# jyakaranda/A-LeGO-LOAM

Measured on AMD Instinct MI355X. Metric: scans/sec (16x1800 LiDAR) full IP->LO->LM loop, higher is better.
Workload: dtype f32/f64

## Files before the change

a-lego-loam_amd/csrc/alego_api.hip:

```cpp
#include <hip/hip_runtime.h>

#include <cmath>
#include <cstdio>
#include <cstdlib>
#include <algorithm>
#include <cstring>
#include <mutex>
#include <set>
#include <string>
#include <vector>

#include "../../include/alego_mi355x.h"
#include "dev_common.h"
#include "dev_mem.h"
#include "front_end.h"
#include "lm_ctx.h"
#include "lm_host.h"
#include "merge_math.h"
#include "thin_math.h"
#include "loop_ctx.h"
#include "pgraph.h"
#include "prof.h"
#include "reloc.h"
#include "stream_plan.h"
// ... 188 lines not shown
  d.cap_sharp = params->n_sharp * params->n_sectors;
  d.cap_lsharp = params->n_less_sharp * params->n_sectors;
  d.cap_flat = params->n_flat * params->n_sectors;
  d.st_stride = d.cap_sharp + d.cap_lsharp + d.cap_flat + d.H;
  d.sin_ax = std::sin(params->seg_alpha_x); d.cos_ax = std::cos(params->seg_alpha_x);
  d.sin_ay = std::sin(params->seg_alpha_y); d.cos_ay = std::cos(params->seg_alpha_y);
  {
    const double lo = params->sensor_mount_ang - params->ground_angle_thres, hi = params->sensor_mount_ang + params->ground_angle_thres;
    const bool ok = lo > -89.0 && hi < 89.0 && lo < hi;
    d.tan_g_lo = ok ? std::tan(lo * M_PI / 180.0) : std::nan("");
    d.tan_g_hi = ok ? std::tan(hi * M_PI / 180.0) : std::nan("");
  }
  d.h_magic = (unsigned)((1ull << 32) / (unsigned long long)d.H) + 1u;
  d.inv_res_x = 1.0 / params->ang_res_x; d.inv_res_y = 1.0 / params->ang_res_y;
  d.tan_theta = (params->seg_theta > 0.0 && params->seg_theta < 1.5) ? std::tan(params->seg_theta) : std::nan("");
  d.opt_ip_fused = env_int("ALEGO_IP_FUSED", 1) != 0;
  d.opt_ip_half = env_int("ALEGO_IP_HALF", 1) != 0;
  d.opt_cc_fused = env_int("ALEGO_CC_FUSED", 1) != 0;
  d.opt_cc_tile = env_int("ALEGO_CC_TILE", 1) != 0;
  d.opt_ip_band = env_int("ALEGO_IP_BAND", 1) != 0;
  d.opt_fe_pick1 = env_int("ALEGO_FE_PICK1", 0) != 0;
  d.opt_fe_fused = env_int("ALEGO_FE_FUSED", 1) != 0;
  d.opt_fe_cand = env_int("ALEGO_FE_CAND", 0);
  d.opt_lo_box_lds = env_int("ALEGO_LO_BOX_LDS", 1 << 20);
  d.opt_lo_grid = env_int("ALEGO_LO_GRID", 1) != 0;
  d.opt_fo_spin = env_int("ALEGO_FE_SPIN", 0);
  d.opt_fo_pad8 = env_int("ALEGO_FE_PAD8", 0) != 0;
  d.opt_map_merge = env_int("ALEGO_MAP_MERGE", 1) != 0;
  d.opt_solve_full_eval = env_int("ALEGO_SOLVE_FULL_EVAL", 0) != 0;
  d.fcap[F_SHARP] = d.cap_sharp * d.NS; d.fcap[F_LSHARP] = d.cap_lsharp * d.NS; d.fcap[F_FLAT] = d.cap_flat * d.NS; d.fcap[F_LFLAT] = d.N;
// ... 714 lines not shown

int alego_debug_check_guards(char* report, int cap) {
  std::string r;
  const int bad = guard_check(&r);
  if (report && cap > 0) { std::strncpy(report, r.c_str(), (size_t)cap - 1); report[cap - 1] = 0; }
  return bad;
}

int alego_debug_set_option(alego_handle* h, const char* name, int value) {
  if (!h || !name) return ALEGO_ERR_ARG;
  const std::string s(name);
  DevCtx& d = h->d;
  if (s == "ALEGO_CC_FUSED") d.opt_cc_fused = value != 0;
  else if (s == "ALEGO_IP_FUSED") d.opt_ip_fused = value != 0;
  else if (s == "ALEGO_IP_HALF") d.opt_ip_half = value != 0;
  else if (s == "ALEGO_CC_TILE") d.opt_cc_tile = value != 0;
  else if (s == "ALEGO_IP_BAND") {
    HIP_TRY(h, hipDeviceSynchronize());
    HIP_TRY(h, hipMemset(d.cc_size, 0, (size_t)d.n_slots * d.N * sizeof(int)));
    HIP_TRY(h, hipMemset(d.cc_rows, 0, (size_t)d.n_slots * d.N * sizeof(unsigned long long)));
    d.opt_ip_band = value != 0;
  }
  else if (s == "ALEGO_FE_PICK1") d.opt_fe_pick1 = value != 0;
  else if (s == "ALEGO_FE_FUSED") d.opt_fe_fused = value != 0;
  else if (s == "ALEGO_FE_CAND") d.opt_fe_cand = value;
  else if (s == "ALEGO_LO_BOX_LDS") d.opt_lo_box_lds = value;
  else if (s == "ALEGO_LO_GRID") d.opt_lo_grid = value != 0;
  else if (s == "ALEGO_FE_SPIN") d.opt_fo_spin = value;
  else if (s == "ALEGO_SOLVE_FULL_EVAL") d.opt_solve_full_eval = value != 0;
  else if (s == "ALEGO_FE_PAD8") d.opt_fo_pad8 = value != 0;
// ... 674 lines not shown
```

a-lego-loam_amd/csrc/dev_common.h:

```cpp
#ifndef ALEGO_DEV_COMMON_H_
#define ALEGO_DEV_COMMON_H_

#include <hip/hip_runtime.h>
#include <stdint.h>

#include "../../include/alego_params.h"
#include "wave.h"

#define IPB_NM 9
#define IP_OWNER_TAG 0x40000000

struct DevCtx {
  alego_params P;
  int n_slots, ring_len;
  int slot0, n_launch;
  int N, H, NS;
  int Pcap;
  int cap_sharp, cap_lsharp, cap_flat;
  double sin_ax, cos_ax, sin_ay, cos_ay;
  double inv_res_x, inv_res_y;
  const double2* ip_rowtab;
  const double2* ip_coltab;
  const double* ip_colfrac;
  int ip_cmin, ip_ncb, ip_fast;
  unsigned h_magic;
  double tan_g_lo, tan_g_hi;
  double tan_theta;
  int opt_ip_fused;
  int opt_ip_half;
  int opt_cc_fused;
  int opt_cc_tile;
  int opt_fe_pick1;
  int opt_fe_fused;
  int opt_fe_cand;
  int opt_lo_box_lds;
  int opt_map_merge;
  int opt_solve_full_eval;
  float4* in_pts;
  int* in_n;
  const float4* bag_pts;
  const int* bag_n;
  const int2* bag_src;
  int n_bags, bag_len, replay_bag;
  int fs_cur, fs_last;
  int* owner;
  float* range_img;
  uint8_t* flag_img;
  int* parent;
  int* cc_size;
  unsigned long long* cc_rows;
  unsigned long long* ipb_col;
// ... 170 lines not shown
```

a-lego-loam_amd/csrc/ip_common.h:

```cpp
#ifndef ALEGO_IP_COMMON_H_
#define ALEGO_IP_COMMON_H_
#include "dev_common.h"

DEV_INLINE int ip_point_cell(const DevCtx& d, const float4 p, bool* valid_out) {
  const alego_params& P = d.P;
  bool valid;
  int cell = -1;
    const bool finite = isfinite(p.x) && isfinite(p.y) && isfinite(p.z);
    valid = finite || P.input_is_dense != 0;
    if (valid && P.near_filter) {
      const float th = (float)P.near_thres;
      if (p.x * p.x + p.y * p.y + p.z * p.z < th * th) valid = false;
    }
    if (valid && finite) {
      int row = -1, col = -1;
      bool slow = true;
      {
        const float h2 = p.x * p.x + p.y * p.y, hf = __builtin_amdgcn_sqrtf(h2);
        bool okr = (d.ip_fast & 1) && hf > 1e-3f && hf < 1e6f && fabsf(p.z) < 1e6f;
        const float t = p.z * __builtin_amdgcn_rcpf(hf), t2 = t * t;
        okr = okr && fabsf(t) < 0.6f;
        const float a = t * (0.99997726f + t2 * (-0.33262347f + t2 * (0.19354346f + t2 * (-0.11643287f + t2 * (0.05265332f + t2 * -0.01172120f)))));
        const float r0 = (a * 57.29577951f + (float)P.ang_bottom) * (float)d.inv_res_y + 0.5f;
        const float kf = floorf(r0);
// ... 142 lines not shown
  }
  const bool live = valid && finite;
  const bool dec = live && c.fast && ok;
  const int row = rfl >= 0 ? rfl : (rfl == -1 ? 0 : -1);
  col = col >= c.H ? col - c.H : col;
  const bool in = row >= 0 && row < c.NS && col >= 0 && col < c.H;
  *valid_out = valid;
  *cell_out = (dec && in) ? col + row * c.H : -1;
  return !live || dec;
}
DEV_INLINE void ip_quick_margins(const DevCtx& d, float* mr, float* mc) {
  *mr = fmaxf(0.005f, 8e-6f * 57.29577951f * (float)d.inv_res_y + 1e-5f);
  *mc = fmaxf(0.02f, 8e-6f * 57.29577951f * (float)d.inv_res_x + 8e-7f * (float)d.H);
}

__device__ __attribute__((noinline)) inline bool ip_is_ground_ref(double dx, double dy, double dz, double mount, double thres) {
  const double angle = (atan2(dz, hypot(dx, dy)) * 180.0) / M_PI;
  return fabs(angle - mount) < thres;
}
__device__ __attribute__((noinline)) inline bool edge_angle_ref(double y, double x, double theta) { return atan2(y, x) > theta; }
DEV_INLINE int ip_ground_margins(double tan_lo, double tan_hi, float fx, float fy, float fz) {
  const double dx = (double)fx, dy = (double)fy, dz = (double)fz;
  const double h2 = dx * dx + dy * dy, z2 = dz * dz;
  const double l2 = (tan_lo * tan_lo) * h2, u2 = (tan_hi * tan_hi) * h2;
  const double sz = copysign(z2, dz);
  const double m1 = sz - copysign(l2, tan_lo), m2 = copysign(u2, tan_hi) - sz;
  const double t1 = 1e-9 * (z2 + l2), t2 = 1e-9 * (z2 + u2);
  const bool yes = m1 > t1 && m2 > t2, no = m1 < -t1 || m2 < -t2;
  return yes ? 1 : (no ? 0 : -1);
}
DEV_INLINE bool ip_is_ground(const DevCtx& d, float fx, float fy, float fz) {
  const int g = ip_ground_margins(d.tan_g_lo, d.tan_g_hi, fx, fy, fz);
  if (g >= 0) return g != 0;
  return ip_is_ground_ref((double)fx, (double)fy, (double)fz, d.P.sensor_mount_ang, d.P.ground_angle_thres);
}

DEV_INLINE int edge_angle_margin(double y, double x, double tan_theta) {
  const double xt = x * tan_theta, m = y - xt;
  return fabs(m) > 1e-9 * (y + fabs(xt)) ? (m > 0.0 ? 1 : 0) : -1;
}
DEV_INLINE bool edge_angle_gt(double y, double x, double theta, double tan_theta) {
  const double xt = x * tan_theta, m = y - xt;
  if (fabs(m) > 1e-9 * (y + fabs(xt))) return m > 0.0;
  return edge_angle_ref(y, x, theta);
}


DEV_INLINE int ccl16_find(uint16_t* par, int v) {
  int curr = par[v];
  if (curr != v) {
    int prev = v, next;
    while (curr > (next = par[curr])) { par[prev] = (uint16_t)next; prev = curr; curr = next; }
  }
  return curr;
}
DEV_INLINE int ccl16_cas(uint16_t* par, int idx, int expect, int val) {
  unsigned* w = reinterpret_cast<unsigned*>(par) + (idx >> 1);
  const int sh = (idx & 1) * 16;
  unsigned old = __hip_atomic_load(w, __ATOMIC_RELAXED, __HIP_MEMORY_SCOPE_WORKGROUP);
// ... 24 lines not shown
```

a-lego-loam_amd/csrc/kernels_ipb.hip:

```cpp
#include <cstdlib>
#include "dev_common.h"
#include "front_end.h"
#include "ip_common.h"
#include "prof.h"

#define IPB_TW 256
#define IPB_NWV (IPB_TW / 64)
#ifndef IPB_MT
#define IPB_MT 512
#endif
#define IPB_LINK_CAP 1024
#define IPB_ET 256
#ifndef IPB_EP
#define IPB_EP 4
#endif

typedef unsigned long long u64;
#ifdef ALEGO_TIMING
__device__ long long ipb_times[48];
extern "C" void alego_ipb_times(long long* out) { (void)hipMemcpyFromSymbol(out, HIP_SYMBOL(ipb_times), sizeof(long long) * 48); }
#define IPB_TICK(k) do { if (threadIdx.x == 0 && blockIdx.x == 0 && blockIdx.y == 0) ipb_times[k] = wall_clock64(); } while (0)
#else
#define IPB_TICK(k)
#endif
DEV_INLINE u64 ipb_low(int r) { return (2ull << r) - 1ull; }
DEV_INLINE int ipb_head(u64 rs, int r) { return 63 - __clzll((long long)(rs & ipb_low(r))); }
DEV_INLINE int ipb_ld(const int* p) { return __hip_atomic_load(p, __ATOMIC_RELAXED, __HIP_MEMORY_SCOPE_AGENT); }
DEV_INLINE u64 ipb_ld64(const u64* p) { return __hip_atomic_load(p, __ATOMIC_RELAXED, __HIP_MEMORY_SCOPE_AGENT); }
DEV_INLINE void ipb_st(int* p, int v) { __hip_atomic_store(p, v, __ATOMIC_RELAXED, __HIP_MEMORY_SCOPE_AGENT); }

DEV_INLINE int ipb_find(int* parent, int v) {
  int curr = ipb_ld(parent + v);
  if (curr != v) {
    int prev = v, next;
    while (curr > (next = ipb_ld(parent + curr))) { ipb_st(parent + prev, next); prev = curr; curr = next; }
  }
  return curr;
}
// ... 3 lines not shown
  return curr;
}
DEV_INLINE int ipb_union(int* parent, int a, int b) {
  int ra = ipb_find(parent, a), rb = ipb_find(parent, b);
  bool repeat;
  int linked = -1;
  do {
    repeat = false;
    if (ra != rb) {
      int ret;
      if (ra < rb) { if ((ret = atomicCAS(parent + rb, rb, ra)) != rb) { rb = ret; repeat = true; } else linked = rb; }
      else { if ((ret = atomicCAS(parent + ra, ra, rb)) != ra) { ra = ret; repeat = true; } else linked = ra; }
    }
  } while (repeat);
  return linked;
}
DEV_INLINE bool ipb_feasible(const alego_params& P, int sz, u64 rows) {
  return sz >= P.seg_big_num || (sz >= P.seg_valid_point_num && (int)__popcll(rows) >= P.seg_valid_line_num);
}

__global__ void __launch_bounds__(IPB_TW) ipb_band(DevCtx d, int ring_pos, int keep) {
  const int slot = blockIdx.y + d.slot0, tid = threadIdx.x, lane = tid & 63, wave = tid >> 6;
  const int H = d.H, NS = d.NS, c0 = blockIdx.x * IPB_TW;
  const int TW = min(IPB_TW, H - c0);
  const bool have = tid < TW;
  const int col = have ? c0 + tid : c0;
  const size_t base = (size_t)slot * d.N;
  const alego_params& P = d.P;
  const float4* pts = scan_pts(d, slot, ring_pos);
  __shared__ uint16_t par[IPB_TW * 64];
// ... 6 lines not shown
    sc[SC_PVALID_OUT] = sc[SC_PVALID];
    sc[SC_FIRST] = 0x7fffffff; sc[SC_LAST] = -1; sc[SC_PVALID] = 0;
    if (last >= 0) {
      const float4 p0 = pts[first], p1 = pts[last];
      float so = -d_atan2f(p0.y, p0.x);
      float eo = (float)((double)(-d_atan2f(p1.y, p1.x)) + 2 * M_PI);
      if ((double)(eo - so) > 3 * M_PI) eo = (float)((double)eo - 2 * M_PI);
      else if ((double)(eo - so) < M_PI) eo = (float)((double)eo + 2 * M_PI);
      ori[0] = so; ori[1] = eo; ori[2] = eo - so;
    }
  }
  IPB_TICK(0);
  int* owner = d.owner + base;
  float rng[64];
  u64 filled = 0, ground = 0;
  {
    float lx = 0, ly = 0, lz = 0;
    bool lower_ok = false;
    int obn[8];
#pragma unroll
    for (int u = 0; u < 8; ++u) obn[u] = (have && u < NS) ? owner[u * H + col] : -1;
#pragma unroll
    for (int row0 = 0; row0 < 64; row0 += 8) {
      if (row0 < NS) {
        int ob[8];
        float4 pb[8];
#pragma unroll
        for (int u = 0; u < 8; ++u) ob[u] = obn[u];
        if (row0 + 8 < 64 && row0 + 8 < NS) {
#pragma unroll
          for (int u = 0; u < 8; ++u) obn[u] = (have && row0 + 8 + u < NS) ? owner[(row0 + 8 + u) * H + col] : -1;
// ... 1 lines not shown
#pragma unroll
        for (int u = 0; u < 8; ++u) {
          ob[u] = (ob[u] >= 0 && (ob[u] & IP_OWNER_TAG)) ? (ob[u] & ~IP_OWNER_TAG) : -1;
          if (have && tid != 0 && row0 + u < NS) owner[(row0 + u) * H + col] = ob[u];
        }
#pragma unroll
        for (int u = 0; u < 8; ++u) pb[u] = pts[max(ob[u], 0)];
#pragma unroll
        for (int u = 0; u < 8; ++u) {
          const int row = row0 + u;
          const bool ok = ob[u] >= 0;
          const float x = pb[u].x, y = pb[u].y, z = pb[u].z;
          const float r = ok ? sqrtf(x * x + y * y + z * z) : -1.0f;
          rng[row] = r;
          if (ok) filled |= 1ull << row;
          if (row >= 1 && row - 1 < P.ground_scan_id && ok && lower_ok) {
            if (ip_is_ground(d, x - lx, y - ly, z - lz)) ground |= 3ull << (row - 1);
          }
          lx = x; ly = y; lz = z; lower_ok = ok;
          if ((keep & 1) && have && row < NS) d.range_img[base + row * H + col] = r;
        }
      } else {
#pragma unroll
        for (int u = 0; u < 8; ++u) rng[row0 + u] = -1.0f;
      }
    }
  }
  IPB_TICK(1);
  const u64 act = filled & ~ground;
  if (have) s_a[tid] = act;
  if (lane == 0) {
#pragma unroll
    for (int row = 0; row < 64; ++row) s_first[wave][row] = rng[row];
  }
  if (wave == 0) {
    const int hc = (c0 + TW == H) ? 0 : c0 + TW;
    int o = lane < NS ? owner[lane * H + hc] : -1;
    o = (o >= 0 && (o & IP_OWNER_TAG)) ? (o & ~IP_OWNER_TAG) : -1;
    const float4 p = pts[max(o, 0)];
    const bool ok = o >= 0;
    const float px = __shfl_up(p.x, 1, 64), py = __shfl_up(p.y, 1, 64), pz = __shfl_up(p.z, 1, 64);
    const int okl = __shfl_up(ok ? 1 : 0, 1, 64);
    bool gp = false;
    if (lane >= 1 && lane - 1 < P.ground_scan_id && ok && okl) gp = ip_is_ground(d, p.x - px, p.y - py, p.z - pz);
    const u64 gb = __ballot(gp), fb = __ballot(ok);
    s_first[IPB_NWV][lane] = ok ? sqrtf(p.x * p.x + p.y * p.y + p.z * p.z) : -1.0f;
    if (lane == 0) s_a[TW] = fb & ~(gb | (gb >> 1));
  }
  __syncthreads();
  IPB_TICK(2);
  u64 ex = 0, ey = 0;
  {
    const u64 act_r = s_a[min(tid + 1, TW)];
    const bool edge_lane = lane == 63 || tid == TW - 1;
    const float* sf = s_first[(tid >= TW - 1) ? IPB_NWV : wave + 1];
#pragma unroll
    for (int row = 0; row < 64; ++row) {
      const float nbd = __int_as_float(__builtin_amdgcn_update_dpp(0, __float_as_int(rng[row]), 0x130, 0xF, 0xF, false));
      const float nbl = sf[row];
      const float nb = edge_lane ? nbl : nbd;
      if ((act >> row) & 1ull) {
        const double r0 = (double)rng[row];
        if ((act_r >> row) & 1ull) {
          const double r1 = (double)nb;
          const double d1 = fmax(r0, r1), d2 = fmin(r0, r1);
          if (edge_angle_gt(d2 * d.sin_ax, d1 - d2 * d.cos_ax, P.seg_theta, d.tan_theta)) ex |= 1ull << row;
        }
        if (row + 1 < 64 && ((act >> (row + 1)) & 1ull)) {
          const double r1 = (double)rng[row + 1 < 64 ? row + 1 : 63];
          const double d1 = fmax(r0, r1), d2 = fmin(r0, r1);
          if (edge_angle_gt(d2 * d.sin_ay, d1 - d2 * d.cos_ay, P.seg_theta, d.tan_theta)) ey |= 1ull << row;
        }
      }
    }
  }
  if (H <= 1) ex = 0;
  IPB_TICK(3);
  const u64 rs = act & ~(ey << 1);
  s_y[tid] = ey; s_rs[tid] = rs;
  for (u64 m = rs; m; m &= m - 1) { const int r = __ffsll((long long)m) - 1; par[r * IPB_TW + tid] = (uint16_t)(r * IPB_TW + tid); }
  __syncthreads();
  IPB_TICK(4);
  if (tid + 1 < TW) {
    const u64 rs_n = s_rs[tid + 1], ey_n = s_y[tid + 1];
    for (u64 m = ex & ~((ex << 1) & (ey << 1) & (ey_n << 1)); m; m &= m - 1) {
      const int r = __ffsll((long long)m) - 1;
// ... 225 lines not shown
```

a-lego-loam_amd/csrc/kernels_ipf.hip:

```cpp
#include <type_traits>
#include <algorithm>
#include <cstdlib>
#include "dev_common.h"
#include "front_end.h"
#include "ip_common.h"
#include "prof.h"

#define IPF2_T 1024
#ifndef IPF_QUICK
#define IPF_QUICK 1
#endif
#define IPF2_NW (IPF2_T / 64)
#define IPF2_ROWS 16

struct IpfShared {
  float first_r[IPF2_NW][IPF2_ROWS];
  unsigned first_act[IPF2_NW];
  int red[3][IPF2_NW];
  int cnt[3][IPF2_ROWS * IPF2_NW];
  int wtot[3][4];
  int tot[3];
  int nlist;
};

#ifdef ALEGO_TIMING
__device__ long long ipf_times[16];
#define IPF_TICK(k) do { if (threadIdx.x == 0 && blockIdx.x == 0) ipf_times[k] = wall_clock64(); } while (0)
extern "C" void alego_ipf_times(long long* out) { (void)hipMemcpyFromSymbol(out, HIP_SYMBOL(ipf_times), sizeof(long long) * 16); }
#else
#define IPF_TICK(k)
#endif

DEV_INLINE int ipf_run_start(unsigned rs, int row) { return 31 - __clz((int)(rs & ((2u << row) - 1u))); }
DEV_INLINE int ipf_run_end(unsigned down, int s) { return s + __ffs((int)~(down >> s)) - 1; }

bool ipf_eligible(const DevCtx& d) { return d.NS <= IPF2_ROWS && (d.H & 1) == 0 && d.H >= 64 && d.H <= 2 * IPF2_T && d.N <= 32768; }
size_t ipf_lds_bytes(const DevCtx& d) { return (size_t)4 * d.N + (size_t)8 * d.H; }

__global__ void __launch_bounds__(IPF2_T) ip_fused(DevCtx d, int ring_pos, int keep) {
  const int slot = blockIdx.x + d.slot0;
  const int tid = threadIdx.x, lane = tid & 63, wave = tid >> 6;
  const int N = d.N, H = d.H, NS = d.NS;
  const size_t base = (size_t)slot * N;
  const alego_params& P = d.P;
  extern __shared__ __attribute__((aligned(16))) unsigned char ipf_smem[];
// ... 422 lines not shown
#else
static size_t iph_pad() { return 0; }
#endif

DEV_INLINE void iph_max16(unsigned* w32, int cell, unsigned val) {
  unsigned* w = w32 + (cell >> 1);
  const int sh = (cell & 1) * 16;
  unsigned old = __hip_atomic_load(w, __ATOMIC_RELAXED, __HIP_MEMORY_SCOPE_WORKGROUP);
  while (((old >> sh) & 0xFFFFu) < val) {
    const unsigned nw = (old & ~(0xFFFFu << sh)) | (val << sh);
    const unsigned got = atomicCAS(w, old, nw);
    if (got == old) break;
    old = got;
  }
}
struct IphCol { unsigned a, b, x, y; };
DEV_INLINE IphCol iph_load(const unsigned long long* fcol, int c) { const unsigned long long v = fcol[c]; IphCol m; m.a = (unsigned)v & 0xFFFFu; m.b = (unsigned)(v >> 16) & 0xFFFFu; m.x = (unsigned)(v >> 32) & 0xFFFFu; m.y = (unsigned)(v >> 48); return m; }
DEV_INLINE void iph_store(unsigned long long* fcol, int c, const IphCol& m) { fcol[c] = (unsigned long long)m.a | ((unsigned long long)m.b << 16) | ((unsigned long long)m.x << 32) | ((unsigned long long)m.y << 48); }

#ifdef IPH_STOP_AFTER
#define IPH_STOP(k) do { if ((k) == IPH_STOP_AFTER) return; } while (0)
#else
#define IPH_STOP(k)
#endif
#ifndef IPH_MINW
#define IPH_MINW 4
#endif
template <int T, int NP>
__global__ void __launch_bounds__(T, IPH_MINW) ip_fused_t(DevCtx d, int ring_pos, int keep) {
  constexpr int NW = T / 64;
  const int slot = blockIdx.x + d.slot0;
  const int tid = threadIdx.x, lane = tid & 63, wave = tid >> 6;
  const int N = d.N, H = d.H, NS = d.NS;
  const size_t base = (size_t)slot * N;
  const alego_params& P = d.P;
  extern __shared__ __attribute__((aligned(16))) unsigned char ipf_smem[];
  unsigned* own16w = reinterpret_cast<unsigned*>(ipf_smem);
  uint16_t* par = reinterpret_cast<uint16_t*>(ipf_smem);
  unsigned long long* fcol = reinterpret_cast<unsigned long long*>(ipf_smem + (size_t)2 * N);
  unsigned* own_g = d.ipf_own + (size_t)slot * (N / 2);
  __shared__ IphShared<NW, NP> S;
  const int hpairs = H / 2;
  IPF_TICK(0);
  for (int v = tid; v < N / 2; v += T) own16w[v] = 0u;
  if (tid == 0) S.nlist = 0;
  __syncthreads();
  const int n = scan_count(d, slot, ring_pos);
  const float4* pts = scan_pts(d, slot, ring_pos);
  { IPH_PHASE_CTX;
  {
// ... 101 lines not shown
      else if ((double)(eo - so) < M_PI) eo = (float)((double)eo + 2 * M_PI);
      ori[0] = so; ori[1] = eo; ori[2] = eo - so;
    }
  }

  }
  IPH_STOP(1);
  IPF_TICK(1);
  { IPH_PHASE_CTX;
#pragma unroll 1
  for (int p = 0; p < NP; ++p) {
    const int pi = tid + p * T, c0 = 2 * pi, c1 = c0 + 1;
    const bool colv = pi < hpairs;
    float rng0[IPF2_ROWS], rng1[IPF2_ROWS];
    unsigned filled0 = 0, filled1 = 0, ground0 = 0, ground1 = 0;
    {
      float lx0 = 0, ly0 = 0, lz0 = 0, lx1 = 0, ly1 = 0, lz1 = 0;
      bool lok0 = false, lok1 = false;
#pragma unroll
      for (int row0 = 0; row0 < IPF2_ROWS; row0 += IPH_GB) {
        unsigned ob[IPH_GB];
        float4 pa[IPH_GB], pb[IPH_GB];
#pragma unroll
        for (int u = 0; u < IPH_GB; ++u) ob[u] = (colv && row0 + u < NS) ? own16w[((row0 + u) * H + c0) >> 1] : 0u;
#pragma unroll
        for (int u = 0; u < IPH_GB; ++u) { pa[u] = pts[max((int)(ob[u] & 0xFFFFu) - 1, 0)]; pb[u] = pts[max((int)(ob[u] >> 16) - 1, 0)]; }
#pragma unroll
        for (int u = 0; u < IPH_GB; ++u) {
          const int row = row0 + u;
          if (colv && row < NS) own_g[(row * H + c0) >> 1] = ob[u];
          {
            const bool ok = (ob[u] & 0xFFFFu) != 0u;
            const float x = pa[u].x, y = pa[u].y, z = pa[u].z;
            rng0[row] = ok ? sqrtf(x * x + y * y + z * z) : -1.0f;
            if (ok) filled0 |= 1u << row;
            if (row >= 1 && row - 1 < P.ground_scan_id && ok && lok0 && ip_is_ground(d, x - lx0, y - ly0, z - lz0)) ground0 |= 3u << (row - 1);
            lx0 = x; ly0 = y; lz0 = z; lok0 = ok;
          }
          {
            const bool ok = (ob[u] >> 16) != 0u;
            const float x = pb[u].x, y = pb[u].y, z = pb[u].z;
            rng1[row] = ok ? sqrtf(x * x + y * y + z * z) : -1.0f;
            if (ok) filled1 |= 1u << row;
            if (row >= 1 && row - 1 < P.ground_scan_id && ok && lok1 && ip_is_ground(d, x - lx1, y - ly1, z - lz1)) ground1 |= 3u << (row - 1);
            lx1 = x; ly1 = y; lz1 = z; lok1 = ok;
          }
        }
      }
    }
    const unsigned act0 = filled0 & ~ground0, act1 = filled1 & ~ground1;
    __syncthreads();
    if (lane == 0) {
#pragma unroll
      for (int r = 0; r < IPF2_ROWS; ++r) S.u.b.first_r[wave][r] = rng0[r];
      S.u.b.first_act[wave] = act0;
    }
    if (p == 0 && tid == 0) {
#pragma unroll
      for (int r = 0; r < IPF2_ROWS; ++r) S.col0_r[r] = rng0[r];
      S.col0_act = act0;
    }
    {
      const int pil = (T - 1) + p * T;
      if (p + 1 < NP && pil < hpairs - 1 && wave == NW - 1 && lane < IPF2_ROWS) {
        const int row = lane, cx = 2 * pil + 2;
        const unsigned ow = row < NS ? (own16w[(row * H + cx) >> 1] & 0xFFFFu) : 0u;
        const float4 q = pts[max((int)ow - 1, 0)];
        const bool ok = ow != 0u;
        const float lx = __shfl_up(q.x, 1, 64), ly = __shfl_up(q.y, 1, 64), lz = __shfl_up(q.z, 1, 64);
        const bool lok = __shfl_up(ok ? 1 : 0, 1, 64) != 0;
        const bool g = row >= 1 && row - 1 < P.ground_scan_id && ok && lok && ip_is_ground(d, q.x - lx, q.y - ly, q.z - lz);
        const unsigned gm = (unsigned)__ballot(g) & 0xFFFFu, fm = (unsigned)__ballot(ok) & 0xFFFFu;
        S.np.np_r[row] = ok ? sqrtf(q.x * q.x + q.y * q.y + q.z * q.z) : -1.0f;
        if (lane == 0) S.np.np_act = fm & ~(gm | (gm >> 1));
      }
    }
    __syncthreads();
    float nbr[IPF2_ROWS];
    unsigned nb_act = (unsigned)__shfl_down((int)act0, 1, 64);
#pragma unroll
    for (int r = 0; r < IPF2_ROWS; ++r) nbr[r] = __shfl_down(rng0[r], 1, 64);
    const bool wrap = pi == hpairs - 1;
    const bool nextpass = !wrap && tid == T - 1 && p + 1 < NP;
    if ((lane == 63 && !nextpass) || wrap) {
      const int sw = min(wave + 1, NW - 1);
#pragma unroll
      for (int r = 0; r < IPF2_ROWS; ++r) nbr[r] = wrap ? S.col0_r[r] : S.u.b.first_r[sw][r];
      nb_act = wrap ? S.col0_act : S.u.b.first_act[sw];
    }
    if (nextpass) {
#pragma unroll
      for (int r = 0; r < IPF2_ROWS; ++r) nbr[r] = S.np.np_r[r];
      nb_act = S.np.np_act;
    }
    unsigned redge0 = 0, redge1 = 0, down0 = 0, down1 = 0;
    if (colv) {
      double k_sax = d.sin_ax, k_cax = d.cos_ax, k_say = d.sin_ay, k_cay = d.cos_ay, k_tan = d.tan_theta, k_theta = P.seg_theta;
      asm volatile("" : "+s"(k_sax), "+s"(k_cax), "+s"(k_say), "+s"(k_cay), "+s"(k_tan), "+s"(k_theta));
#pragma unroll
      for (int row = 0; row < IPF2_ROWS; ++row) {
        if (row < NS) {
          if ((act0 >> row) & 1u) {
            const double r0 = (double)rng0[row];
            if ((act1 >> row) & 1u) {
              const double r1 = (double)rng1[row], d1 = fmax(r0, r1), d2 = fmin(r0, r1);
              if (edge_angle_gt(d2 * k_sax, d1 - d2 * k_cax, k_theta, k_tan)) redge0 |= 1u << row;
            }
            if (row + 1 < NS && ((act0 >> (row + 1)) & 1u)) {
              const double r1 = (double)rng0[row + 1 < IPF2_ROWS ? row + 1 : row], d1 = fmax(r0, r1), d2 = fmin(r0, r1);
              if (edge_angle_gt(d2 * k_say, d1 - d2 * k_cay, k_theta, k_tan)) down0 |= 1u << row;
            }
          }
          if ((act1 >> row) & 1u) {
            const double r0 = (double)rng1[row];
            if ((nb_act >> row) & 1u) {
              const double r1 = (double)nbr[row], d1 = fmax(r0, r1), d2 = fmin(r0, r1);
              if (edge_angle_gt(d2 * k_sax, d1 - d2 * k_cax, k_theta, k_tan)) redge1 |= 1u << row;
            }
            if (row + 1 < NS && ((act1 >> (row + 1)) & 1u)) {
              const double r1 = (double)rng1[row + 1 < IPF2_ROWS ? row + 1 : row], d1 = fmax(r0, r1), d2 = fmin(r0, r1);
              if (edge_angle_gt(d2 * k_say, d1 - d2 * k_cay, k_theta, k_tan)) down1 |= 1u << row;
            }
          }
        }
      }
      fcol[c0] = (unsigned long long)ground0 | ((unsigned long long)act0 << 16) | ((unsigned long long)redge0 << 32) | ((unsigned long long)down0 << 48);
      fcol[c1] = (unsigned long long)ground1 | ((unsigned long long)act1 << 16) | ((unsigned long long)redge1 << 32) | ((unsigned long long)down1 << 48);
      if (keep & 1) {
        float* rimg = d.range_img + base;
        uint8_t* fimg = d.flag_img + base;
#pragma unroll
        for (int row = 0; row < IPF2_ROWS; ++row) {
          if (row < NS) {
            rimg[row * H + c0] = rng0[row]; rimg[row * H + c1] = rng1[row];
            fimg[row * H + c0] = (uint8_t)(((ground0 >> row) & 1u) | (((act0 >> row) & 1u) << 1) | (((redge0 >> row) & 1u) << 2) | (((down0 >> row) & 1u) << 3));
            fimg[row * H + c1] = (uint8_t)(((ground1 >> row) & 1u) | (((act1 >> row) & 1u) << 1) | (((redge1 >> row) & 1u) << 2) | (((down1 >> row) & 1u) << 3));
          }
        }
      }
    }
// ... 305 lines not shown
```

Measured before the change: 480,300.

## Screen ground and edge-angle tests in fp32 with exact fp64 fallback

Replaces the per-cell fp64 ground-angle and edge-angle predicates in the image-projection kernels with fp32 screening tests built from host-precomputed constants and error bands. Cells the screen cannot decide confidently are collected in bitmasks and re-evaluated with the original fp64/atan2 path, reloading their points from the owner map. The aim is to cut fp64 arithmetic and divergent branching in the hot unrolled row loops, at the cost of a second, gather-based slow pass for ambiguous cells and extra register pressure.

```diff
diff --git a/a-lego-loam_amd/csrc/alego_api.hip b/a-lego-loam_amd/csrc/alego_api.hip
--- a/a-lego-loam_amd/csrc/alego_api.hip
+++ b/a-lego-loam_amd/csrc/alego_api.hip
@@ -226,6 +226,8 @@
   d.h_magic = (unsigned)((1ull << 32) / (unsigned long long)d.H) + 1u;
   d.inv_res_x = 1.0 / params->ang_res_x; d.inv_res_y = 1.0 / params->ang_res_y;
   d.tan_theta = (params->seg_theta > 0.0 && params->seg_theta < 1.5) ? std::tan(params->seg_theta) : std::nan("");
+  d.opt_ip_screen = env_int("ALEGO_IP_SCREEN", 1) != 0;
+  d.ip_scr = ip_screen_consts(d.sin_ax, d.cos_ax, d.sin_ay, d.cos_ay, d.tan_theta, d.tan_g_lo, d.tan_g_hi, d.opt_ip_screen);
   d.opt_ip_fused = env_int("ALEGO_IP_FUSED", 1) != 0;
   d.opt_ip_half = env_int("ALEGO_IP_HALF", 1) != 0;
   d.opt_cc_fused = env_int("ALEGO_CC_FUSED", 1) != 0;
@@ -970,6 +972,7 @@
   if (s == "ALEGO_CC_FUSED") d.opt_cc_fused = value != 0;
   else if (s == "ALEGO_IP_FUSED") d.opt_ip_fused = value != 0;
   else if (s == "ALEGO_IP_HALF") d.opt_ip_half = value != 0;
+  else if (s == "ALEGO_IP_SCREEN") { d.opt_ip_screen = value != 0; d.ip_scr = ip_screen_consts(d.sin_ax, d.cos_ax, d.sin_ay, d.cos_ay, d.tan_theta, d.tan_g_lo, d.tan_g_hi, d.opt_ip_screen); }
   else if (s == "ALEGO_CC_TILE") d.opt_cc_tile = value != 0;
   else if (s == "ALEGO_IP_BAND") {
     HIP_TRY(h, hipDeviceSynchronize());
diff --git a/a-lego-loam_amd/csrc/dev_common.h b/a-lego-loam_amd/csrc/dev_common.h
--- a/a-lego-loam_amd/csrc/dev_common.h
+++ b/a-lego-loam_amd/csrc/dev_common.h
@@ -6,6 +6,7 @@
 
 #include "../../include/alego_params.h"
 #include "wave.h"
+#include "ip_pred.h"
 
 #define IPB_NM 9
 #define IP_OWNER_TAG 0x40000000
@@ -26,6 +27,7 @@
   unsigned h_magic;
   double tan_g_lo, tan_g_hi;
   double tan_theta;
+  IpScreenConsts ip_scr;
   int opt_ip_fused;
   int opt_ip_half;
   int opt_cc_fused;
@@ -35,6 +37,7 @@
   int opt_fe_cand;
   int opt_lo_box_lds;
   int opt_map_merge;
+  int opt_ip_screen;
   int opt_solve_full_eval;
   float4* in_pts;
   int* in_n;
diff --git a/a-lego-loam_amd/csrc/ip_common.h b/a-lego-loam_amd/csrc/ip_common.h
--- a/a-lego-loam_amd/csrc/ip_common.h
+++ b/a-lego-loam_amd/csrc/ip_common.h
@@ -180,35 +180,8 @@
   *mc = fmaxf(0.02f, 8e-6f * 57.29577951f * (float)d.inv_res_x + 8e-7f * (float)d.H);
 }
 
-__device__ __attribute__((noinline)) inline bool ip_is_ground_ref(double dx, double dy, double dz, double mount, double thres) {
-  const double angle = (atan2(dz, hypot(dx, dy)) * 180.0) / M_PI;
-  return fabs(angle - mount) < thres;
-}
-__device__ __attribute__((noinline)) inline bool edge_angle_ref(double y, double x, double theta) { return atan2(y, x) > theta; }
-DEV_INLINE int ip_ground_margins(double tan_lo, double tan_hi, float fx, float fy, float fz) {
-  const double dx = (double)fx, dy = (double)fy, dz = (double)fz;
-  const double h2 = dx * dx + dy * dy, z2 = dz * dz;
-  const double l2 = (tan_lo * tan_lo) * h2, u2 = (tan_hi * tan_hi) * h2;
-  const double sz = copysign(z2, dz);
-  const double m1 = sz - copysign(l2, tan_lo), m2 = copysign(u2, tan_hi) - sz;
-  const double t1 = 1e-9 * (z2 + l2), t2 = 1e-9 * (z2 + u2);
-  const bool yes = m1 > t1 && m2 > t2, no = m1 < -t1 || m2 < -t2;
-  return yes ? 1 : (no ? 0 : -1);
-}
 DEV_INLINE bool ip_is_ground(const DevCtx& d, float fx, float fy, float fz) {
-  const int g = ip_ground_margins(d.tan_g_lo, d.tan_g_hi, fx, fy, fz);
-  if (g >= 0) return g != 0;
-  return ip_is_ground_ref((double)fx, (double)fy, (double)fz, d.P.sensor_mount_ang, d.P.ground_angle_thres);
-}
-
-DEV_INLINE int edge_angle_margin(double y, double x, double tan_theta) {
-  const double xt = x * tan_theta, m = y - xt;
-  return fabs(m) > 1e-9 * (y + fabs(xt)) ? (m > 0.0 ? 1 : 0) : -1;
-}
-DEV_INLINE bool edge_angle_gt(double y, double x, double theta, double tan_theta) {
-  const double xt = x * tan_theta, m = y - xt;
-  if (fabs(m) > 1e-9 * (y + fabs(xt))) return m > 0.0;
-  return edge_angle_ref(y, x, theta);
+  return ip_ground_decide(d.tan_g_lo, d.tan_g_hi, d.P.sensor_mount_ang, d.P.ground_angle_thres, fx, fy, fz);
 }
 
 
diff --git a/a-lego-loam_amd/csrc/ip_pred.h b/a-lego-loam_amd/csrc/ip_pred.h
--- /dev/null
+++ b/a-lego-loam_amd/csrc/ip_pred.h
@@ -0,0 +1,106 @@
+#ifndef ALEGO_IP_PRED_H_
+#define ALEGO_IP_PRED_H_
+
+#ifdef __HIPCC__
+#define IP_PRED_FN __device__ __forceinline__
+#define IP_PRED_REF __device__ __attribute__((noinline)) inline
+#define IP_PRED_HOST __host__ inline
+#else
+#include <math.h>
+#define IP_PRED_FN inline
+#define IP_PRED_REF inline
+#define IP_PRED_HOST inline
+#endif
+
+IP_PRED_REF bool ip_is_ground_ref(double dx, double dy, double dz, double mount, double thres) {
+  const double angle = (atan2(dz, hypot(dx, dy)) * 180.0) / M_PI;
+  return fabs(angle - mount) < thres;
+}
+IP_PRED_REF bool edge_angle_ref(double y, double x, double theta) { return atan2(y, x) > theta; }
+IP_PRED_FN int ip_ground_margins(double tan_lo, double tan_hi, float fx, float fy, float fz) {
+  const double dx = (double)fx, dy = (double)fy, dz = (double)fz;
+  const double h2 = dx * dx + dy * dy, z2 = dz * dz;
+  const double l2 = (tan_lo * tan_lo) * h2, u2 = (tan_hi * tan_hi) * h2;
+  const double sz = copysign(z2, dz);
+  const double m1 = sz - copysign(l2, tan_lo), m2 = copysign(u2, tan_hi) - sz;
+  const double t1 = 1e-9 * (z2 + l2), t2 = 1e-9 * (z2 + u2);
+  const bool yes = m1 > t1 && m2 > t2, no = m1 < -t1 || m2 < -t2;
+  return yes ? 1 : (no ? 0 : -1);
+}
+IP_PRED_FN bool ip_ground_decide(double tan_lo, double tan_hi, double mount, double thres, float fx, float fy, float fz) {
+  const int g = ip_ground_margins(tan_lo, tan_hi, fx, fy, fz);
+  if (g >= 0) return g != 0;
+  return ip_is_ground_ref((double)fx, (double)fy, (double)fz, mount, thres);
+}
+
+IP_PRED_FN int edge_angle_margin(double y, double x, double tan_theta) {
+  const double xt = x * tan_theta, m = y - xt;
+  return fabs(m) > 1e-9 * (y + fabs(xt)) ? (m > 0.0 ? 1 : 0) : -1;
+}
+IP_PRED_FN bool edge_angle_gt(double y, double x, double theta, double tan_theta) {
+  const double xt = x * tan_theta, m = y - xt;
+  if (fabs(m) > 1e-9 * (y + fabs(xt))) return m > 0.0;
+  return edge_angle_ref(y, x, theta);
+}
+
+struct IpScreenBits { bool yes, und; };
+
+#define IP_SCREEN_TINY 1e-24f
+IP_PRED_FN IpScreenBits ip_edge_screen(float d1, float d2, float kh, float kl, float band) {
+  const float p = d2 * kh, e = fmaf(d2, kh, -p), s = p - d1, E = s + fmaf(d2, kl, e);
+  const bool dec = fabsf(E) > band * d1 && d2 >= IP_SCREEN_TINY;
+  IpScreenBits r;
+  r.yes = dec && E > 0.0f;
+  r.und = !dec;
+  return r;
+}
+
+#define IP_GROUND_TOL 4e-6f
+#define IP_GROUND_FLOOR 1e-30f
+IP_PRED_FN IpScreenBits ip_ground_screen(float g_lo, float g_hi, float g_max, float fx, float fy, float fz) {
+  const float h2 = fx * fx + fy * fy, z2 = fz * fz;
+  const float sz = copysignf(z2, fz);
+  const float m1 = sz - g_lo * h2, m2 = g_hi * h2 - sz;
+  const float sum = z2 + g_max * h2, tol = IP_GROUND_TOL * sum;
+  const bool big = sum >= IP_GROUND_FLOOR;
+  const bool yes = m1 > tol && m2 > tol, no = m1 < -tol || m2 < -tol;
+  IpScreenBits r;
+  r.yes = yes && big;
+  r.und = !((yes || no) && big);
+  return r;
+}
+
+struct IpScreenConsts {
+  float kxh, kxl, kyh, kyl;
+  float eband;
+  float g_lo, g_hi, g_max;
+};
+IP_PRED_HOST double ip_edge_band(double sin_a, double cos_a, double tan_theta) {
+  if (!(tan_theta > 0.0) || !(tan_theta < 1e3) || !(sin_a > 0.0) || !(cos_a > 0.0) || !(sin_a < 1.0)) return -1.0;
+  const double K = (sin_a + cos_a * tan_theta) / tan_theta;
+  if (!(K > 1.0 / 1024.0) || !(K < 1024.0)) return -1.0;
+  const double b = 4.0 * (2.01e-9 * sin_a / tan_theta + 1e-15 * (1.0 + 1.0 / tan_theta) + 2.9e-14);
+  if (!(b < 1e-6)) return -1.0;
+  return b > 8e-9 ? b : 8e-9;
+}
+IP_PRED_HOST IpScreenConsts ip_screen_consts(double sin_ax, double cos_ax, double sin_ay, double cos_ay, double tan_theta, double tan_lo, double tan_hi, int enable) {
+  IpScreenConsts c;
+  c.kxh = c.kxl = c.kyh = c.kyl = NAN; c.eband = INFINITY;
+  c.g_lo = c.g_hi = c.g_max = NAN;
+  if (!enable) return c;
+  const double bx = ip_edge_band(sin_ax, cos_ax, tan_theta), by = ip_edge_band(sin_ay, cos_ay, tan_theta);
+  if (bx > 0.0 && by > 0.0) {
+    const double Kx = (sin_ax + cos_ax * tan_theta) / tan_theta, Ky = (sin_ay + cos_ay * tan_theta) / tan_theta;
+    c.kxh = (float)Kx; c.kxl = (float)(Kx - (double)c.kxh);
+    c.kyh = (float)Ky; c.kyl = (float)(Ky - (double)c.kyh);
+    c.eband = (float)((bx > by ? bx : by) * (1.0 + 1e-6));
+  }
+  if (tan_lo < tan_hi && fabs(tan_lo) < 1e3 && fabs(tan_hi) < 1e3) {
+    const double l2 = tan_lo * tan_lo, u2 = tan_hi * tan_hi;
+    c.g_lo = (float)copysign(l2, tan_lo); c.g_hi = (float)copysign(u2, tan_hi);
+    c.g_max = (float)((l2 > u2 ? l2 : u2) * (1.0 + 1e-6));
+  }
+  return c;
+}
+
+#endif
diff --git a/a-lego-loam_amd/csrc/kernels_ipb.hip b/a-lego-loam_amd/csrc/kernels_ipb.hip
--- a/a-lego-loam_amd/csrc/kernels_ipb.hip
+++ b/a-lego-loam_amd/csrc/kernels_ipb.hip
@@ -20,8 +20,15 @@
 __device__ long long ipb_times[48];
 extern "C" void alego_ipb_times(long long* out) { (void)hipMemcpyFromSymbol(out, HIP_SYMBOL(ipb_times), sizeof(long long) * 48); }
 #define IPB_TICK(k) do { if (threadIdx.x == 0 && blockIdx.x == 0 && blockIdx.y == 0) ipb_times[k] = wall_clock64(); } while (0)
+__device__ unsigned long long ipb_slow_cnt[4];
+#define IPB_SLOW_COUNT(k) do { if ((threadIdx.x & 63) == 0) atomicAdd(&ipb_slow_cnt[k], 1ull); } while (0)
+extern "C" void alego_ipb_slow_counts(unsigned long long* out, int reset) {
+  (void)hipMemcpyFromSymbol(out, HIP_SYMBOL(ipb_slow_cnt), sizeof(unsigned long long) * 4);
+  if (reset) { const unsigned long long z[4] = {0, 0, 0, 0}; (void)hipMemcpyToSymbol(HIP_SYMBOL(ipb_slow_cnt), z, sizeof(z)); }
+}
 #else
 #define IPB_TICK(k)
+#define IPB_SLOW_COUNT(k)
 #endif
 DEV_INLINE u64 ipb_low(int r) { return (2ull << r) - 1ull; }
 DEV_INLINE int ipb_head(u64 rs, int r) { return 63 - __clzll((long long)(rs & ipb_low(r))); }
@@ -55,6 +62,11 @@
     }
   } while (repeat);
   return linked;
+}
+DEV_INLINE float4 ipb_cell_point(const int* owner, const float4* pts, int H, int row, int col) { return pts[max(ipb_ld(owner + row * H + col), 0) & ~IP_OWNER_TAG]; }
+DEV_INLINE float ipb_cell_range(const int* owner, const float4* pts, int H, int row, int col) {
+  const float4 q = ipb_cell_point(owner, pts, H, row, col);
+  return sqrtf(q.x * q.x + q.y * q.y + q.z * q.z);
 }
 DEV_INLINE bool ipb_feasible(const alego_params& P, int sz, u64 rows) {
   return sz >= P.seg_big_num || (sz >= P.seg_valid_point_num && (int)__popcll(rows) >= P.seg_valid_line_num);
@@ -91,7 +103,11 @@
   int* owner = d.owner + base;
   float rng[64];
   u64 filled = 0, ground = 0;
+  IPB_SLOW_COUNT(0);
   {
+    float k_glo = d.ip_scr.g_lo, k_ghi = d.ip_scr.g_hi, k_gmax = d.ip_scr.g_max;
+    asm volatile("" : "+s"(k_glo), "+s"(k_ghi), "+s"(k_gmax));
+    u64 gund = 0;
     float lx = 0, ly = 0, lz = 0;
     bool lower_ok = false;
     int obn[8];
@@ -123,8 +139,11 @@
           const float r = ok ? sqrtf(x * x + y * y + z * z) : -1.0f;
           rng[row] = r;
           if (ok) filled |= 1ull << row;
-          if (row >= 1 && row - 1 < P.ground_scan_id && ok && lower_ok) {
-            if (ip_is_ground(d, x - lx, y - ly, z - lz)) ground |= 3ull << (row - 1);
+          if (row >= 1 && row - 1 < P.ground_scan_id) {
+            const IpScreenBits g = ip_ground_screen(k_glo, k_ghi, k_gmax, x - lx, y - ly, z - lz);
+            const bool en = ok && lower_ok;
+            ground |= (en && g.yes) ? 3ull << (row - 1) : 0ull;
+            gund |= (en && g.und) ? 1ull << row : 0ull;
           }
           lx = x; ly = y; lz = z; lower_ok = ok;
           if ((keep & 1) && have && row < NS) d.range_img[base + row * H + col] = r;
@@ -132,6 +151,15 @@
       } else {
 #pragma unroll
         for (int u = 0; u < 8; ++u) rng[row0 + u] = -1.0f;
+      }
+    }
+    if (__ballot(gund != 0ull)) {
+      IPB_SLOW_COUNT(1);
+#pragma unroll 1
+      for (u64 m = gund; m; m &= m - 1) {
+        const int row = __ffsll((long long)m) - 1;
+        const float4 q = ipb_cell_point(owner, pts, H, row, col), l = ipb_cell_point(owner, pts, H, row - 1, col);
+        if (ip_is_ground(d, q.x - l.x, q.y - l.y, q.z - l.z)) ground |= 3ull << (row - 1);
       }
     }
   }
@@ -150,8 +178,12 @@
     const bool ok = o >= 0;
     const float px = __shfl_up(p.x, 1, 64), py = __shfl_up(p.y, 1, 64), pz = __shfl_up(p.z, 1, 64);
     const int okl = __shfl_up(ok ? 1 : 0, 1, 64);
-    bool gp = false;
-    if (lane >= 1 && lane - 1 < P.ground_scan_id && ok && okl) gp = ip_is_ground(d, p.x - px, p.y - py, p.z - pz);
+    const IpScreenBits gs = ip_ground_screen(d.ip_scr.g_lo, d.ip_scr.g_hi, d.ip_scr.g_max, p.x - px, p.y - py, p.z - pz);
+    const bool gen = lane >= 1 && lane - 1 < P.ground_scan_id && ok && okl;
+    bool gp = gen && gs.yes;
+    if (__ballot(gen && gs.und)) {
+      if (gen && gs.und) gp = ip_is_ground(d, p.x - px, p.y - py, p.z - pz);
+    }
     const u64 gb = __ballot(gp), fb = __ballot(ok);
     s_first[IPB_NWV][lane] = ok ? sqrtf(p.x * p.x + p.y * p.y + p.z * p.z) : -1.0f;
     if (lane == 0) s_a[TW] = fb & ~(gb | (gb >> 1));
@@ -163,22 +195,42 @@
     const u64 act_r = s_a[min(tid + 1, TW)];
     const bool edge_lane = lane == 63 || tid == TW - 1;
     const float* sf = s_first[(tid >= TW - 1) ? IPB_NWV : wave + 1];
+    float k_kxh = d.ip_scr.kxh, k_kxl = d.ip_scr.kxl, k_kyh = d.ip_scr.kyh, k_kyl = d.ip_scr.kyl, k_eb = d.ip_scr.eband;
+    asm volatile("" : "+s"(k_kxh), "+s"(k_kxl), "+s"(k_kyh), "+s"(k_kyl), "+s"(k_eb));
+    u64 ux = 0, uy = 0;
 #pragma unroll
     for (int row = 0; row < 64; ++row) {
       const float nbd = __int_as_float(__builtin_amdgcn_update_dpp(0, __float_as_int(rng[row]), 0x130, 0xF, 0xF, false));
       const float nbl = sf[row];
       const float nb = edge_lane ? nbl : nbd;
-      if ((act >> row) & 1ull) {
-        const double r0 = (double)rng[row];
-        if ((act_r >> row) & 1ull) {
-          const double r1 = (double)nb;
+      const float r0 = rng[row];
+      if (__ballot((act >> row) & 1ull)) {
+        {
+          const IpScreenBits e = ip_edge_screen(fmaxf(r0, nb), fminf(r0, nb), k_kxh, k_kxl, k_eb);
+          ex |= e.yes ? 1ull << row : 0ull; ux |= e.und ? 1ull << row : 0ull;
+        }
+        if (row + 1 < 64) {
+          const float r1 = rng[row + 1 < 64 ? row + 1 : 63];
+          const IpScreenBits e = ip_edge_screen(fmaxf(r0, r1), fminf(r0, r1), k_kyh, k_kyl, k_eb);
+          ey |= e.yes ? 1ull << row : 0ull; uy |= e.und ? 1ull << row : 0ull;
+        }
+      }
+    }
+    const u64 sx = act & act_r, sy = act & (act >> 1);
+    ex &= sx; ey &= sy; ux &= sx; uy &= sy;
+    if (__ballot((ux | uy) != 0ull)) {
+      IPB_SLOW_COUNT(2);
+      const int cr = col + 1 == H ? 0 : col + 1;
+#pragma unroll 1
+      for (int k = 0; k < 2; ++k) {
+        const double sa = k ? d.sin_ay : d.sin_ax, ca = k ? d.cos_ay : d.cos_ax;
+#pragma unroll 1
+        for (u64 m = k ? uy : ux; m; m &= m - 1) {
+          const int row = __ffsll((long long)m) - 1;
+          const double r0 = (double)ipb_cell_range(owner, pts, H, row, col);
+          const double r1 = (double)(k ? ipb_cell_range(owner, pts, H, row + 1, col) : ipb_cell_range(owner, pts, H, row, cr));
           const double d1 = fmax(r0, r1), d2 = fmin(r0, r1);
-          if (edge_angle_gt(d2 * d.sin_ax, d1 - d2 * d.cos_ax, P.seg_theta, d.tan_theta)) ex |= 1ull << row;
-        }
-        if (row + 1 < 64 && ((act >> (row + 1)) & 1ull)) {
-          const double r1 = (double)rng[row + 1 < 64 ? row + 1 : 63];
-          const double d1 = fmax(r0, r1), d2 = fmin(r0, r1);
-          if (edge_angle_gt(d2 * d.sin_ay, d1 - d2 * d.cos_ay, P.seg_theta, d.tan_theta)) ey |= 1ull << row;
+          if (edge_angle_gt(d2 * sa, d1 - d2 * ca, P.seg_theta, d.tan_theta)) { if (k) ey |= 1ull << row; else ex |= 1ull << row; }
         }
       }
     }
diff --git a/a-lego-loam_amd/csrc/kernels_ipf.hip b/a-lego-loam_amd/csrc/kernels_ipf.hip
--- a/a-lego-loam_amd/csrc/kernels_ipf.hip
+++ b/a-lego-loam_amd/csrc/kernels_ipf.hip
@@ -27,8 +27,15 @@
 __device__ long long ipf_times[16];
 #define IPF_TICK(k) do { if (threadIdx.x == 0 && blockIdx.x == 0) ipf_times[k] = wall_clock64(); } while (0)
 extern "C" void alego_ipf_times(long long* out) { (void)hipMemcpyFromSymbol(out, HIP_SYMBOL(ipf_times), sizeof(long long) * 16); }
+__device__ unsigned long long iph_slow_cnt[4];
+#define IPH_SLOW_COUNT(k) do { if ((threadIdx.x & 63) == 0) atomicAdd(&iph_slow_cnt[k], 1ull); } while (0)
+extern "C" void alego_iph_slow_counts(unsigned long long* out, int reset) {
+  (void)hipMemcpyFromSymbol(out, HIP_SYMBOL(iph_slow_cnt), sizeof(unsigned long long) * 4);
+  if (reset) { const unsigned long long z[4] = {0, 0, 0, 0}; (void)hipMemcpyToSymbol(HIP_SYMBOL(iph_slow_cnt), z, sizeof(z)); }
+}
 #else
 #define IPF_TICK(k)
+#define IPH_SLOW_COUNT(k)
 #endif
 
 DEV_INLINE int ipf_run_start(unsigned rs, int row) { return 31 - __clz((int)(rs & ((2u << row) - 1u))); }
@@ -481,6 +488,14 @@
     old = got;
   }
 }
+DEV_INLINE float4 iph_cell_point(const unsigned* own16w, const float4* pts, int H, int row, int col) {
+  const unsigned ow = (own16w[(row * H + col) >> 1] >> ((col & 1) * 16)) & 0xFFFFu;
+  return pts[max((int)ow - 1, 0)];
+}
+DEV_INLINE float iph_cell_range(const unsigned* own16w, const float4* pts, int H, int row, int col) {
+  const float4 q = iph_cell_point(own16w, pts, H, row, col);
+  return sqrtf(q.x * q.x + q.y * q.y + q.z * q.z);
+}
 struct IphCol { unsigned a, b, x, y; };
 DEV_INLINE IphCol iph_load(const unsigned long long* fcol, int c) { const unsigned long long v = fcol[c]; IphCol m; m.a = (unsigned)v & 0xFFFFu; m.b = (unsigned)(v >> 16) & 0xFFFFu; m.x = (unsigned)(v >> 32) & 0xFFFFu; m.y = (unsigned)(v >> 48); return m; }
 DEV_INLINE void iph_store(unsigned long long* fcol, int c, const IphCol& m) { fcol[c] = (unsigned long long)m.a | ((unsigned long long)m.b << 16) | ((unsigned long long)m.x << 32) | ((unsigned long long)m.y << 48); }
@@ -500,7 +515,6 @@
   const int tid = threadIdx.x, lane = tid & 63, wave = tid >> 6;
   const int N = d.N, H = d.H, NS = d.NS;
   const size_t base = (size_t)slot * N;
-  const alego_params& P = d.P;
   extern __shared__ __attribute__((aligned(16))) unsigned char ipf_smem[];
   unsigned* own16w = reinterpret_cast<unsigned*>(ipf_smem);
   uint16_t* par = reinterpret_cast<uint16_t*>(ipf_smem);
@@ -632,7 +646,11 @@
     const bool colv = pi < hpairs;
     float rng0[IPF2_ROWS], rng1[IPF2_ROWS];
     unsigned filled0 = 0, filled1 = 0, ground0 = 0, ground1 = 0;
+    IPH_SLOW_COUNT(0);
     {
+      float k_glo = d.ip_scr.g_lo, k_ghi = d.ip_scr.g_hi, k_gmax = d.ip_scr.g_max;
+      asm volatile("" : "+s"(k_glo), "+s"(k_ghi), "+s"(k_gmax));
+      unsigned gund = 0;
       float lx0 = 0, ly0 = 0, lz0 = 0, lx1 = 0, ly1 = 0, lz1 = 0;
       bool lok0 = false, lok1 = false;
 #pragma unroll
@@ -652,7 +670,12 @@
             const float x = pa[u].x, y = pa[u].y, z = pa[u].z;
             rng0[row] = ok ? sqrtf(x * x + y * y + z * z) : -1.0f;
             if (ok) filled0 |= 1u << row;
-            if (row >= 1 && row - 1 < P.ground_scan_id && ok && lok0 && ip_is_ground(d, x - lx0, y - ly0, z - lz0)) ground0 |= 3u << (row - 1);
+            if (row >= 1 && row - 1 < P.ground_scan_id) {
+              const IpScreenBits g = ip_ground_screen(k_glo, k_ghi, k_gmax, x - lx0, y - ly0, z - lz0);
+              const bool en = ok && lok0;
+              ground0 |= (en && g.yes) ? 3u << (row - 1) : 0u;
+              gund |= (en && g.und) ? 1u << row : 0u;
+            }
             lx0 = x; ly0 = y; lz0 = z; lok0 = ok;
           }
           {
@@ -660,9 +683,23 @@
             const float x = pb[u].x, y = pb[u].y, z = pb[u].z;
             rng1[row] = ok ? sqrtf(x * x + y * y + z * z) : -1.0f;
             if (ok) filled1 |= 1u << row;
-            if (row >= 1 && row - 1 < P.ground_scan_id && ok && lok1 && ip_is_ground(d, x - lx1, y - ly1, z - lz1)) ground1 |= 3u << (row - 1);
+            if (row >= 1 && row - 1 < P.ground_scan_id) {
+              const IpScreenBits g = ip_ground_screen(k_glo, k_ghi, k_gmax, x - lx1, y - ly1, z - lz1);
+              const bool en = ok && lok1;
+              ground1 |= (en && g.yes) ? 3u << (row - 1) : 0u;
+              gund |= (en && g.und) ? 0x10000u << row : 0u;
+            }
             lx1 = x; ly1 = y; lz1 = z; lok1 = ok;
           }
+        }
+      }
+      if (__ballot(gund != 0u)) {
+        IPH_SLOW_COUNT(1);
+#pragma unroll 1
+        for (unsigned m = gund; m; m &= m - 1) {
+          const int b = __ffs((int)m) - 1, row = b & 15, c = c0 + (b >> 4);
+          const float4 q = iph_cell_point(own16w, pts, H, row, c), l = iph_cell_point(own16w, pts, H, row - 1, c);
+          if (ip_is_ground(d, q.x - l.x, q.y - l.y, q.z - l.z)) { if (b >> 4) ground1 |= 3u << (row - 1); else ground0 |= 3u << (row - 1); }
         }
       }
     }
@@ -687,7 +724,12 @@
         const bool ok = ow != 0u;
         const float lx = __shfl_up(q.x, 1, 64), ly = __shfl_up(q.y, 1, 64), lz = __shfl_up(q.z, 1, 64);
         const bool lok = __shfl_up(ok ? 1 : 0, 1, 64) != 0;
-        const bool g = row >= 1 && row - 1 < P.ground_scan_id && ok && lok && ip_is_ground(d, q.x - lx, q.y - ly, q.z - lz);
+        const IpScreenBits gs = ip_ground_screen(d.ip_scr.g_lo, d.ip_scr.g_hi, d.ip_scr.g_max, q.x - lx, q.y - ly, q.z - lz);
+        const bool gen = row >= 1 && row - 1 < P.ground_scan_id && ok && lok;
+        bool g = gen && gs.yes;
+        if (__ballot(gen && gs.und)) {
+          if (gen && gs.und) g = ip_is_ground(d, q.x - lx, q.y - ly, q.z - lz);
+        }
         const unsigned gm = (unsigned)__ballot(g) & 0xFFFFu, fm = (unsigned)__ballot(ok) & 0xFFFFu;
         S.np.np_r[row] = ok ? sqrtf(q.x * q.x + q.y * q.y + q.z * q.z) : -1.0f;
         if (lane == 0) S.np.np_act = fm & ~(gm | (gm >> 1));
@@ -712,36 +754,62 @@
       nb_act = S.np.np_act;
     }
     unsigned redge0 = 0, redge1 = 0, down0 = 0, down1 = 0;
+    unsigned ux0 = 0, ux1 = 0, uy0 = 0, uy1 = 0;
     if (colv) {
-      double k_sax = d.sin_ax, k_cax = d.cos_ax, k_say = d.sin_ay, k_cay = d.cos_ay, k_tan = d.tan_theta, k_theta = P.seg_theta;
-      asm volatile("" : "+s"(k_sax), "+s"(k_cax), "+s"(k_say), "+s"(k_cay), "+s"(k_tan), "+s"(k_theta));
+      float k_kxh = d.ip_scr.kxh, k_kxl = d.ip_scr.kxl, k_kyh = d.ip_scr.kyh, k_kyl = d.ip_scr.kyl, k_eb = d.ip_scr.eband;
+      asm volatile("" : "+s"(k_kxh), "+s"(k_kxl), "+s"(k_kyh), "+s"(k_kyl), "+s"(k_eb));
 #pragma unroll
       for (int row = 0; row < IPF2_ROWS; ++row) {
-        if (row < NS) {
-          if ((act0 >> row) & 1u) {
-            const double r0 = (double)rng0[row];
-            if ((act1 >> row) & 1u) {
-              const double r1 = (double)rng1[row], d1 = fmax(r0, r1), d2 = fmin(r0, r1);
-              if (edge_angle_gt(d2 * k_sax, d1 - d2 * k_cax, k_theta, k_tan)) redge0 |= 1u << row;
+        if (row < NS && __ballot(((act0 | act1) >> row) & 1u)) {
+          const float a0 = rng0[row], a1 = rng1[row];
+          {
+            const IpScreenBits e = ip_edge_screen(fmaxf(a0, a1), fminf(a0, a1), k_kxh, k_kxl, k_eb);
+            redge0 |= e.yes ? 1u << row : 0u; ux0 |= e.und ? 1u << row : 0u;
+          }
+          {
+            const float nb = nbr[row];
+            const IpScreenBits e = ip_edge_screen(fmaxf(a1, nb), fminf(a1, nb), k_kxh, k_kxl, k_eb);
+            redge1 |= e.yes ? 1u << row : 0u; ux1 |= e.und ? 1u << row : 0u;
+          }
+          if (row + 1 < IPF2_ROWS) {
+            const float b0 = rng0[row + 1 < IPF2_ROWS ? row + 1 : row], b1 = rng1[row + 1 < IPF2_ROWS ? row + 1 : row];
+            const IpScreenBits e = ip_edge_screen(fmaxf(a0, b0), fminf(a0, b0), k_kyh, k_kyl, k_eb);
+            down0 |= e.yes ? 1u << row : 0u; uy0 |= e.und ? 1u << row : 0u;
+            const IpScreenBits f = ip_edge_screen(fmaxf(a1, b1), fminf(a1, b1), k_kyh, k_kyl, k_eb);
+            down1 |= f.yes ? 1u << row : 0u; uy1 |= f.und ? 1u << row : 0u;
+          }
+        }
+      }
+      {
+        const unsigned sx0 = act0 & act1, sx1 = act1 & nb_act, sy0 = act0 & (act0 >> 1), sy1 = act1 & (act1 >> 1);
+        redge0 &= sx0; redge1 &= sx1; down0 &= sy0; down1 &= sy1;
+        ux0 &= sx0; ux1 &= sx1; uy0 &= sy0; uy1 &= sy1;
+      }
+    }
+    {
+      const unsigned und_x = ux0 | (ux1 << 16), und_y = uy0 | (uy1 << 16);
+      if (__ballot((und_x | und_y) != 0u)) {
+        IPH_SLOW_COUNT(2);
+        const double theta = P.seg_theta, tan_theta = d.tan_theta;
+#pragma unroll 1
+        for (int k = 0; k < 2; ++k) {
+          const double sa = k ? d.sin_ay : d.sin_ax, ca = k ? d.cos_ay : d.cos_ax;
+#pragma unroll 1
+          for (unsigned m = k ? und_y : und_x; m; m &= m - 1) {
+            const int b = __ffs((int)m) - 1, row = b & 15, c = c0 + (b >> 4);
+            const int cr = c + 1 == H ? 0 : c + 1;
+            const double r0 = (double)iph_cell_range(own16w, pts, H, row, c);
+            const double r1 = (double)(k ? iph_cell_range(own16w, pts, H, row + 1, c) : iph_cell_range(own16w, pts, H, row, cr));
+            const double d1 = fmax(r0, r1), d2 = fmin(r0, r1);
+            if (edge_angle_gt(d2 * sa, d1 - d2 * ca, theta, tan_theta)) {
+              const unsigned bit = 1u << row;
+              if (k) { if (b >> 4) down1 |= bit; else down0 |= bit; } else { if (b >> 4) redge1 |= bit; else redge0 |= bit; }
             }
-            if (row + 1 < NS && ((act0 >> (row + 1)) & 1u)) {
-              const double r1 = (double)rng0[row + 1 < IPF2_ROWS ? row + 1 : row], d1 = fmax(r0, r1), d2 = fmin(r0, r1);
-              if (edge_angle_gt(d2 * k_say, d1 - d2 * k_cay, k_theta, k_tan)) down0 |= 1u << row;
-            }
-          }
-          if ((act1 >> row) & 1u) {
-            const double r0 = (double)rng1[row];
-            if ((nb_act >> row) & 1u) {
-              const double r1 = (double)nbr[row], d1 = fmax(r0, r1), d2 = fmin(r0, r1);
-              if (edge_angle_gt(d2 * k_sax, d1 - d2 * k_cax, k_theta, k_tan)) redge1 |= 1u << row;
-            }
-            if (row + 1 < NS && ((act1 >> (row + 1)) & 1u)) {
-              const double r1 = (double)rng1[row + 1 < IPF2_ROWS ? row + 1 : row], d1 = fmax(r0, r1), d2 = fmin(r0, r1);
-              if (edge_angle_gt(d2 * k_say, d1 - d2 * k_cay, k_theta, k_tan)) down1 |= 1u << row;
-            }
-          }
-        }
-      }
+          }
+        }
+      }
+    }
+    if (colv) {
       fcol[c0] = (unsigned long long)ground0 | ((unsigned long long)act0 << 16) | ((unsigned long long)redge0 << 32) | ((unsigned long long)down0 << 48);
       fcol[c1] = (unsigned long long)ground1 | ((unsigned long long)act1 << 16) | ((unsigned long long)redge1 << 32) | ((unsigned long long)down1 << 48);
       if (keep & 1) {
```

New measurement: 485,900, median of 6. 1.2% higher.
